# michaelwfc/distributed-tensorflow-resnet

Hardware: AMD Instinct MI355X
Metric: steps/sec (global_batch=128 CIFAR-10 / 1024 ImageNet) ResNet-50 at 1/2/4/8 MI355X (higher is better)
Workload: dtype bf16; 1 GPU; model=resnet50_v2_cifar10, global_batch=128, per_gpu_batch=128, image_size=32, parallelism=dp1, allreduce_dtype=fp32, roctx=False, device=AMD Radeon Graphics, graph=False, wgrad_stream=False, persist_overlap=False, cus=256

## Files before the change

distributed_tensorflow_resnet_amd/csrc/prn_bwd.hip:

```cpp
#include "prn_device.h"

namespace dtr {

namespace {

__device__ __forceinline__ WLoad wl_dgrad(const bf16* src, int co, int ci, int ks) {
  const int K = ks * ks * co;
  return WLoad{src, ci, K, kpad_of(K), 1, ci, co, __frcp_rn((float)(K / 8)), __builtin_ctz(co / 8),
               __builtin_ctz(ci)};
}

template <int SO, int P, int CO, bool PROJ>
__device__ __forceinline__ void dgrad_s2_acc(f32x4 (&acc)[8], const bf16* hal, const bf16* wl,
                                             int kslice, int wave, int lane) {
  using G = Stg<SO, P>;
  lane = opaque_v(lane);
  static_assert(G::CLS, "class-major output");
  if (!wave_active<SO, P>(wave)) return;
  constexpr int RL = G::R / 2, RSL = G::RS / 2, W2L = RL + 2, UL = CO / 8;
  constexpr int KP = kpad_of(PROJ ? CO : 9 * CO);
  const int fr = lane & 15, fq = lane >> 4;
  int pb0, cb0;
  tile_of<SO, P>(wave, 0, pb0, cb0);
  const int cls = (pb0 * 16) / (G::NPX / 4);
// ... 45 lines not shown
                lds16(hal + haddr<G::U>(lr * G::W2 + lc, lc, u * 8)));
  }
}

__device__ __forceinline__ void bn_prefetch_bwd(const PrnBn& bn, int C, BnRegs& r) {
  const int c = threadIdx.x;
  if (c < C) {
    r.g = ldg(bn.gamma + c);
    r.mean = ldg(bn.mean + c);
    r.rstd = ldg(bn.rstd + c);
    r.scale = ldg(bn.scale + c);
    r.shift = ldg(bn.shift + c);
  }
}

__device__ __forceinline__ void bn_prefetch_tab(const PrnBn& bn, int C, BnRegs& r) {
  const int c = threadIdx.x;
  if (c < C) {
    r.scale = ldg(bn.scale + c);
    r.shift = ldg(bn.shift + c);
    r.mean = ldg(bn.mean + c);
    r.rstd = ldg(bn.rstd + c);
  }
}
__device__ __forceinline__ void tab_store(const BnRegs& r, int C, float* tbl) {
  const int c = threadIdx.x;
  if (c < C) {
    tbl[c] = r.scale;
    tbl[64 + c] = r.shift;
    tbl[128 + c] = -r.mean * r.rstd;
    tbl[192 + c] = r.rstd;
  }
}

__device__ __forceinline__ void bn_bwd_table(const PrnBn& bn, const BnRegs& pr, int C, float M,
                                             float* tbl) {
  const int c = threadIdx.x;
  if (c < C) {
    double d1, d2;
    acc_read(bn.bacc, C, c, d1, d2);
    const float sg = (float)d1, sgx = (float)d2;
    const float a = pr.g * pr.rstd;
    const float b = a * sg / M, cc = a * sgx / M;
    tbl[c] = a;
    tbl[64 + c] = cc * pr.mean * pr.rstd - b;
    tbl[128 + c] = -cc * pr.rstd;
    tbl[192 + c] = pr.scale;
    tbl[256 + c] = pr.shift;
    if (blockIdx.x == 0) {
      st_sc1_f32(bn.dbeta + c, sg);
      st_sc1_f32(bn.dgamma + c, sgx);
    }
  }
  __syncthreads();
}

__device__ __forceinline__ void bn_load_table(const PrnBn& bn, int C, float* tbl) {
  const int c = threadIdx.x;
  if (c < C) {
    const float rs = ldg(bn.rstd + c);
    tbl[c] = ldg(bn.scale + c);
    tbl[64 + c] = ldg(bn.shift + c);
    tbl[128 + c] = -ldg(bn.mean + c) * rs;
    tbl[192 + c] = rs;
  }
}

__device__ __forceinline__ float bwd1(float da, float xf, const float* cf, int c) {
  const float gg = fmaf(xf, cf[192 + c], cf[256 + c]) > 0.f ? da : 0.f;
  return fmaf(cf[128 + c], xf, fmaf(cf[c], gg, cf[64 + c]));
}
__device__ __forceinline__ bf16x8 bwd8(bf16x8 da, bf16x8 x, bf16x8 add, bool has_add,
                                       const float* cf, int c0) {
  bf16x8 o;
#pragma unroll
  for (int j = 0; j < 8; ++j) {
    float r = bwd1((float)da[j], (float)x[j], cf, c0 + j);
    if (has_add) r += (float)add[j];
    o[j] = (bf16)r;
  }
  return o;
}

__device__ __forceinline__ void arrive_bwd(Ctx& x) {
  grid_arrive(x.a->bar + PRN_BWD, x.a->shards);
  if (x.mark != nullptr) {
    if (threadIdx.x == 0) __hip_atomic_fetch_add(x.mark, 1u, __ATOMIC_RELAXED, __HIP_MEMORY_SCOPE_AGENT);
    x.mark = nullptr;
  }
}
__device__ __forceinline__ bool wait_bwd(Ctx& x) {
  ++x.nbar;
  const bool ok = grid_wait(x.a->bar, PRN_BWD, x.nbar, x.slices, x.a->shards, x.a->err, x.m.flag);
  if (ok && blockIdx.x == 0 && threadIdx.x == 0)
    __hip_atomic_store(x.a->bar + PRN_READY, x.nbar, __ATOMIC_RELAXED, __HIP_MEMORY_SCOPE_AGENT);
  return ok;
}

template <int S, int P>
__device__ __forceinline__ void bwd_sums(Ctx& x, const bf16x4 (&da)[8], const bf16x4 (&xs)[8],
                                         const float* tb, int bi, int wave, int lane) {
  lane = opaque_v(lane);
  bn_sums<S, P>([&](int t, int r, float& s1, float& s2) {
    int pb, cb;
    tile_of<S, P>(wave, t, pb, cb);
    const int c = cb * 16 + 4 * (lane >> 4) + r;
    const float xf = (float)xs[t][r];
    const float gg = (xf * tb[c] + tb[64 + c] > 0.f) ? (float)da[t][r] : 0.f;
    s1 = gg;
    s2 = gg * fmaf(xf, tb[192 + c], tb[128 + c]);
  }, x.m.red, ld_const(x.a->bns + (bi)).bacc, wave, lane);
}

template <int S, int P, bool ADD>
__device__ __forceinline__ void bwd_apply(bf16x4 (&out)[8], const bf16x4 (&da)[8],
                                          const bf16x4 (&xs)[8], const bf16x4 (&add)[8],
                                          const float* cf, int wave, int lane) {
  lane = opaque_v(lane);
  if (!wave_active<S, P>(wave)) return;
#pragma unroll
  for (int t = 0; t < Stg<S, P>::TPW; ++t) {
    int pb, cb;
    tile_of<S, P>(wave, t, pb, cb);
#pragma unroll
    for (int r = 0; r < 4; ++r) {
      const int c = cb * 16 + 4 * (lane >> 4) + r;
      float o = bwd1((float)da[t][r], (float)xs[t][r], cf, c);
      if (ADD) o += (float)add[t][r];
      out[t][r] = (bf16)o;
    }
  }
}

struct NbrBwd {
  bf16x8 dv, xv, av;
};
template <int S, int P>
__device__ __forceinline__ void bwd_nbr_issue(const Nbr<S, P>& nb, const bf16* da,
                                              const bf16* xsrc, const bf16* add, NbrBwd& q) {
  if ((int)threadIdx.x < Nbr<S, P>::UNITS && nb.ok) {
    q.dv = da ? ld_sc1_b128(da, nb.gofs) : bf16x8{};
    q.xv = ldg(reinterpret_cast<const bf16x8*>(xsrc + nb.gofs));
    q.av = add ? ld_sc1_b128(add, nb.gofs) : bf16x8{};
  }
}
template <int S, int P>
__device__ __forceinline__ void bwd_halo(Ctx& x, bf16* hal, const bf16x4 (&own)[8],
                                         const Nbr<S, P>& nb, NbrBwd& q, const float* dpc,
                                         bool has_add, const float* cf, int wave, int lane) {
  bf16x8 nv = {};
  if ((int)threadIdx.x < Nbr<S, P>::UNITS && nb.ok) {
    if (dpc) {
#pragma unroll
      for (int j = 0; j < 8; ++j) q.dv[j] = (bf16)dpc[nb.u * 8 + j];
    }
    nv = bwd8(q.dv, q.xv, q.av, has_add, cf, nb.u * 8);
  }
  to_halo<S, P, 0>(hal, own, nullptr, nullptr, nb, nv, x.kslice, wave, lane);
}

template <int S, int STR, bool PROJ, int P>
__device__ __forceinline__ bool block_bwd(Ctx& x, bf16x4 (&dout)[8], bf16x4 (&hs)[8],
                                          const WLoad& next_w2, bool has_prev,
                                          const PrnBlock& Bn, const PrnBlock& B) {
  constexpr int SI = STR == 2 ? S - 1 : S;
  using GI = Stg<SI, P>;
  using G = Stg<S, P>;
  const PrnArgs& a = *x.a;
  const int wave = opaque_s(x.wave), lane = opaque_v(x.lane);
  const long img_o = (long)x.img * G::R * G::R * G::C;
  const long img_i = (long)x.img * GI::R * GI::R * GI::C;
  probe(x, 100 + S);
  bf16x4 xs[8];
  load_regs<SI, P>(xs, B.x + img_i, x.kslice, wave, lane);
  tab_store(x.ftr, G::C, x.m.tbl);
  __syncthreads();
  probe(x, 1);
  f32x4 acc[8];
  zero_acc(acc);
  conv_acc<S, P, G::C, 3, 1, true>(acc, x.m.hb, x.m.w1, x.kslice, wave, lane, x.m.red);
  bf16x4 da[8];
  round_acc<S, P, false>(da, acc, da);
  probe(x, 3);
  if constexpr (P > 1)
    publish<S, P, 1>(da, B.da2 + img_o, x.kslice, wave, lane);
  bwd_sums<S, P>(x, da, hs, x.m.tbl, B.bn2, wave, lane);
  probe(x, 4);
  arrive_bwd(x);
  {
    const WLoad L1 = wl_dgrad(B.w1b, G::C, GI::C, 3);
    WLoad LP{};
    if (PROJ) LP = wl_dgrad(B.wpb, G::C, GI::C, 1);
    bf16x8 w1r[nreg(conv_units(G::C, GI::C, 3))], wpr[1];
    w_prefetch(L1, w1r);
    w_prefetch(LP, wpr);
    bn_prefetch_bwd(ld_const(a.bns + (B.bn2)), G::C, x.bnr);
    bn_prefetch_tab(ld_const(a.bns + (B.bn1)), GI::C, x.ftr);
    halo_to_global<S, P>(x.m.hb, B.dout + img_o, x.kslice);
    probe(x, 5);
    if (!wait_bwd(x)) return false;
    probe(x, 6);
    const Nbr<S, P> nb(x.kslice);
    NbrBwd q;
    bwd_nbr_issue<S, P>(nb, B.da2 + img_o, B.h1 + img_o, nullptr, q);
    bn_bwd_table(ld_const(a.bns + (B.bn2)), x.bnr, G::C, (float)a.N * G::R * G::R, x.m.tbl2);
    bf16x4 dh[8];
    bwd_apply<S, P, false>(dh, da, hs, dh, x.m.tbl2, wave, lane);
    bwd_halo<S, P>(x, x.m.ha, dh, nb, q, nullptr, false, x.m.tbl2, wave, lane);
    tab_store(x.ftr, GI::C, x.m.tbl);
    w_store(L1, w1r, x.m.w1);
    w_store(LP, wpr, x.m.w2);
  }
  __syncthreads();
  probe(x, 8);
  zero_acc(acc);
  if constexpr (STR == 2) {
    dgrad_s2_acc<SI, P, G::C, false>(acc, x.m.ha, x.m.w1, x.kslice, wave, lane);
    dgrad_s2_acc<SI, P, G::C, true>(acc, x.m.hb, x.m.w2, x.kslice, wave, lane);
  } else {
    conv_acc<S, P, G::C, 3, 1, true>(acc, x.m.ha, x.m.w1, x.kslice, wave, lane, x.m.red);
    if constexpr (PROJ) conv_acc<S, P, G::C, 1, 1, false>(acc, x.m.hb, x.m.w2, x.kslice, wave, lane, x.m.red);
  }
  round_acc<SI, P, false>(da, acc, da);
  probe(x, 9);
  if constexpr (P > 1)
    publish<SI, P, 1>(da, B.da1 + img_i, x.kslice, wave, lane);
  bwd_sums<SI, P>(x, da, xs, x.m.tbl, B.bn1, wave, lane);
  probe(x, 10);
  arrive_bwd(x);
  halo_to_global<S, P>(x.m.ha, B.dh1 + img_o, x.kslice);
  probe(x, 11);
  bf16x8 w2r[nreg(conv_units(G::C, G::C, 3))];
  w_prefetch(next_w2, w2r);
  bn_prefetch_bwd(ld_const(a.bns + (B.bn1)), GI::C, x.bnr);
  if (has_prev) bn_prefetch_tab(ld_const(a.bns + (Bn.bn2)), GI::C, x.ftr);
  if (!wait_bwd(x)) return false;
  probe(x, 12);
  const Nbr<SI, P> nb(x.kslice);
  NbrBwd q;
  bwd_nbr_issue<SI, P>(nb, B.da1 + img_i, B.x + img_i, PROJ ? nullptr : B.dout + img_o, q);
  bn_bwd_table(ld_const(a.bns + (B.bn1)), x.bnr, GI::C, (float)a.N * GI::R * GI::R, x.m.tbl2);
  probe(x, 13);
  if (PROJ && a.overlap && blockIdx.x == 0 && a.bucket_of_stage[S] >= 0)
    x.mark = a.bar + PRN_BUCKET + a.bucket_of_stage[S] * PRN_LINE;
  if constexpr (PROJ) bwd_apply<SI, P, false>(dout, da, xs, dout, x.m.tbl2, wave, lane);
  else bwd_apply<SI, P, true>(dout, da, xs, dout, x.m.tbl2, wave, lane);
  probe(x, 14);
  if (has_prev) load_regs<SI, P>(hs, Bn.h1 + img_i, x.kslice, wave, lane);
  bwd_halo<SI, P>(x, x.m.hb, dout, nb, q, nullptr, !PROJ, x.m.tbl2, wave, lane);
  probe(x, 15);
  w_store(next_w2, w2r, x.m.w1);
  return true;
}

template <int CO, int CI, int KSZ, int STR, int RO, int WT>
__device__ __forceinline__ void wgrad_item(const PrnItem& it, char* smem, int wave, int lane, bool wt) {
  constexpr int RI = RO * STR, W2 = RI + 2, OFF = KSZ == 1 ? 1 : 0;
  constexpr int KN = KSZ * KSZ * CI, NB = (KN + 15) / 16, MB = CO / 16;
  constexpr int TILES = MB * NB, TPW = TILES / WT, WKS = NW / WT;
  constexpr int KSI = RO * RO / 32, KPW = KSI / WKS;
  static_assert(TILES % WT == 0 && KSI % WKS == 0 && TPW <= 36, "wgrad tiles");
  static_assert(NB % TPW == 0, "a wave's tiles share one output-channel block");
  bf16* dys = reinterpret_cast<bf16*>(smem);
  bf16* hal = dys + RO * RO * CO;
  float* tb = reinterpret_cast<float*>(hal + W2 * W2 * CI);
  const int tid = threadIdx.x;
  wave = opaque_s(wave);
  lane = opaque_v(lane);
  const int tg = wave % WT, kq = wave / WT;
  const int gq = lane >> 4, li = lane & 15, qr = li >> 2, pc = li & 3;
  if (it.scale != nullptr && tid < CI) {
    tb[tid] = ldg(it.scale + tid);
    tb[64 + tid] = ldg(it.shift + tid);
  }
  f32x4 acc[TPW];
#pragma unroll
  for (int t = 0; t < TPW; ++t) acc[t] = f32x4{0.f, 0.f, 0.f, 0.f};
  constexpr int DU = RO * RO * CO / 8, CU = CI / 8, XU = W2 * W2 * CU;
  constexpr int ND = (DU + PT - 1) / PT, NX = (XU + PT - 1) / PT;
  bf16x8 rd[ND], rx[NX];
  auto fetch = [&](int n) {
#pragma unroll
    for (int i = 0; i < ND; ++i) {
      const int q = tid + i * PT;
      if (q < DU) rd[i] = ld_sc1_b128(it.dy, (long)n * RO * RO * CO + q * 8);
    }
#pragma unroll
    for (int i = 0; i < NX; ++i) {
      const int q = tid + i * PT, pix = q / CU, u = q - pix * CU;
      const int hr = pix / W2, hc = pix - hr * W2;
      rx[i] = bf16x8{};
      if (q < XU && hr >= 1 && hr <= RI && hc >= 1 && hc <= RI)
        rx[i] = ldg(reinterpret_cast<const bf16x8*>(it.x + (((long)n * RI + hr - 1) * RI + hc - 1) * CI + u * 8));
    }
  };
  const int nend = it.img0 + it.nimg;
  fetch(it.img0);
  for (int n = it.img0; n < nend; ++n) {
    __syncthreads();
#pragma unroll
    for (int i = 0; i < ND; ++i) {
      const int q = tid + i * PT;
      if (q < DU) *reinterpret_cast<bf16x8*>(dys + q * 8) = rd[i];
    }
#pragma unroll
    for (int i = 0; i < NX; ++i) {
      const int q = tid + i * PT, pix = q / CU, u = q - pix * CU;
      const int hr = pix / W2, hc = pix - hr * W2;
      if (q < XU) {
        bf16x8 v = rx[i];
        if (it.scale != nullptr && hr >= 1 && hr <= RI && hc >= 1 && hc <= RI)
          v = affine_relu8(v, tb + u * 8, tb + 64 + u * 8);
// ... 57 lines not shown
    for (int t = 0; t < TPW; ++t) {
      const int tile = tg * TPW + t, mb = tile / NB, nb = tile - mb * NB;
      const int n = nb * 16 + li;
      if (n < KN) {
        if (wt) {
#pragma unroll
          for (int i = 0; i < 4; ++i) st_sc1_f32(it.part + (long)(mb * 16 + 4 * gq + i) * KN + n, acc[t][i]);
        } else {
#pragma unroll
          for (int i = 0; i < 4; ++i) stg(it.part + (long)(mb * 16 + 4 * gq + i) * KN + n, acc[t][i]);
        }
      }
    }
  }
  __syncthreads();
}

constexpr int PRN_KINDS = 9;
__host__ __device__ constexpr int wg_lds(int co, int ci, int str, int ro) {
  return ro * ro * co * 2 + (ro * str + 2) * (ro * str + 2) * ci * 2 + 512;
}

__device__ __forceinline__ void run_item(const PrnItem& it, char* smem, int wave, int lane, bool wt) {
  switch (it.kind) {
    case 0: wgrad_item<16, 16, 3, 1, 32, 1>(it, smem, wave, lane, wt); break;
    case 1: wgrad_item<32, 32, 3, 1, 16, 2>(it, smem, wave, lane, wt); break;
    case 2: wgrad_item<64, 64, 3, 1, 8, 8>(it, smem, wave, lane, wt); break;
    case 3: wgrad_item<32, 16, 3, 2, 16, 2>(it, smem, wave, lane, wt); break;
    case 4: wgrad_item<64, 32, 3, 2, 8, 8>(it, smem, wave, lane, wt); break;
    case 5: wgrad_item<16, 16, 1, 1, 32, 1>(it, smem, wave, lane, wt); break;
    case 6: wgrad_item<32, 16, 1, 2, 16, 2>(it, smem, wave, lane, wt); break;
    case 7: wgrad_item<64, 32, 1, 2, 8, 8>(it, smem, wave, lane, wt); break;
    case 8: wgrad_item<16, 8, 3, 1, 32, 1>(it, smem, wave, lane, wt); break;
    default: break;
  }
}


}

template <int P>
__device__ __forceinline__ bool prn_bwd_slices(const PrnArgs& a, char* smem, int wave, int lane) {
  const int nsl = a.N * P;
  const int tid = threadIdx.x;
  Ctx x;
  x.a = &a;
  x.m = carve(smem);
  x.img = blockIdx.x / P;
  x.kslice = blockIdx.x % P;
  x.wave = wave;
  x.lane = lane;
  x.nbar = 0;
  x.slices = (unsigned)nsl;
  x.pc = 0;
  x.mark = nullptr;
  probe(x, 0);
  const int nb = a.nblocks;
  const PrnBlock& BL = ld_const(a.blocks + (nb - 1));
  {
    const WLoad L = wl_dgrad(BL.w2b, 64, 64, 3);
    bf16x8 r[nreg(conv_units(64, 64, 3))];
    w_prefetch(L, r);
    w_store(L, r, x.m.w1);
  }
  using G2 = Stg<2, P>;
  bf16x4 dout[8], hs[8];
  {
    const int fb = 2 * nb;
    const long img_o = (long)x.img * 64 * 64;
    bf16x4 xs[8];
    load_regs<2, P>(xs, BL.out + img_o, x.kslice, wave, lane);
    float* dps = x.m.tbl + 256;
    bn_load_table(ld_const(a.bns + (fb)), 64, x.m.tbl);
    if (tid < 64) dps[tid] = a.dpool[(long)x.img * 64 + tid];
    __syncthreads();
    bf16x4 dp[8];
#pragma unroll
    for (int t = 0; t < G2::TPW; ++t) {
      int pb, cb;
      tile_of<2, P>(wave, t, pb, cb);
#pragma unroll
      for (int r = 0; r < 4; ++r) dp[t][r] = (bf16)dps[(cb * 16 + 4 * (lane >> 4) + r) & 63];
    }
    bwd_sums<2, P>(x, dp, xs, x.m.tbl, fb, wave, lane);
    arrive_bwd(x);
    bn_prefetch_bwd(ld_const(a.bns + (fb)), 64, x.bnr);
    bn_prefetch_tab(ld_const(a.bns + (BL.bn2)), 64, x.ftr);
    if (!wait_bwd(x)) return false;
    const Nbr<2, P> nb(x.kslice);
    NbrBwd q;
    bwd_nbr_issue<2, P>(nb, nullptr, BL.out + img_o, nullptr, q);
    bn_bwd_table(ld_const(a.bns + (fb)), x.bnr, 64, (float)a.N * 64, x.m.tbl2);
    bwd_apply<2, P, false>(dout, dp, xs, dout, x.m.tbl2, wave, lane);
    load_regs<2, P>(hs, BL.h1 + img_o, x.kslice, wave, lane);
    bwd_halo<2, P>(x, x.m.hb, dout, nb, q, dps, false, x.m.tbl2, wave, lane);
  }
  const int nps = nb / 3;
  auto run = [&](auto tag, int bi) -> bool {
    constexpr int S = decltype(tag)::S, STR = decltype(tag)::STR;
    constexpr bool PROJ = decltype(tag)::PROJ;
    WLoad n2{};
    const bool hp = bi > 0;
    const PrnBlock Bp = ld_const(a.blocks + (hp ? bi - 1 : bi));
    if (hp) n2 = wl_dgrad(Bp.w2b, 16 << Bp.stage, 16 << Bp.stage, 3);
    return block_bwd<S, STR, PROJ, P>(x, dout, hs, n2, hp, Bp, ld_const(a.blocks + (bi)));
  };
  for (int bi = nb - 1; bi > 2 * nps; --bi)
    if (!run(BlkTag<2, 1, false>{}, bi)) return false;
  if (!run(BlkTag<2, 2, true>{}, 2 * nps)) return false;
  for (int bi = 2 * nps - 1; bi > nps; --bi)
    if (!run(BlkTag<1, 1, false>{}, bi)) return false;
  if (!run(BlkTag<1, 2, true>{}, nps)) return false;
  for (int bi = nps - 1; bi > 0; --bi)
    if (!run(BlkTag<0, 1, false>{}, bi)) return false;
  if (!run(BlkTag<0, 1, true>{}, 0)) return false;
  probe(x, 200);
  if constexpr (P == 1) {
    __syncthreads();
    halo_to_global<0, P>(x.m.hb, a.dx0 + (long)x.img * 1024 * 16, x.kslice);
  } else {
    publish<0, P>(dout, a.dx0 + (long)x.img * 1024 * 16, x.kslice, wave, lane);
  }
  arrive_bwd(x);
  if (blockIdx.x == 0) wait_bwd(x);
  return true;
}

__device__ void prn_head_fold(const PrnArgs& a, char* smem, int tid) {
  const int N = a.N, ld = a.kpad, classes = a.classes;
  float* red = reinterpret_cast<float*>(smem);
  float* sw = red + 256;
  bf16* sp = reinterpret_cast<bf16*>(sw + ((N * ld + 3 * N + 3) & ~3));
  bf16* sd = sp + N * 64;
  for (int i = tid; i < N * ld / 4; i += PT)
    reinterpret_cast<f32x4*>(sw)[i] = ldg(reinterpret_cast<const f32x4*>(a.ws) + i);
  for (int i = tid; i < N; i += PT)
    reinterpret_cast<float2*>(sw + N * ld)[i] = ldg(reinterpret_cast<const float2*>(a.ws + N * ld) + i);
  if (a.topk_out != nullptr)
    for (int i = tid; i < N; i += PT) sw[N * ld + 2 * N + i] = ldg(a.ws + N * ld + 2 * N + i);
  for (int i = tid; i < N * 8; i += PT)
    reinterpret_cast<uint4*>(sp)[i] = ldg(reinterpret_cast<const uint4*>(a.pooled) + i);
  for (int i = tid; i < N * ld / 8; i += PT)
    reinterpret_cast<uint4*>(sd)[i] = ldg(reinterpret_cast<const uint4*>(a.dlogits) + i);
  __syncthreads();
  const int lane = tid & 63, q = tid >> 6;
  if (q < 4) {
    float t = 0.f;
    if (lane < classes) {
#pragma unroll 8
      for (int r = q; r < N; r += 4) t += sw[r * ld + lane];
    }
    red[q * 64 + lane] = t;
  } else if (q == 4) {
    const float* rs = sw + N * ld;
    float l = 0.f, k = 0.f;
    for (int r = lane; r < N; r += 64) {
      l += rs[2 * r];
      k += rs[2 * r + 1];
    }
    l = wave_sum(l);
    k = wave_sum(k);
    if (lane == 0) {
      stg(a.loss_sum, l);
      stg(a.correct, k);
    }
    if (a.topk_out != nullptr) {
      const float* rk = rs + 2 * N;
      float k5 = 0.f;
// ... 164 lines not shown
```

distributed_tensorflow_resnet_amd/csrc/prn_device.h:

```cpp
#pragma once
#include <algorithm>
#include <stdexcept>

#include "common.h"
#include "kernels.h"

namespace dtr {

namespace {

constexpr int PT = PRN_THREADS;
constexpr int NW = PT / 64;
constexpr long long kSpinTicks = 200000000;

typedef unsigned u32x2 __attribute__((ext_vector_type(2)));
typedef unsigned u32x4 __attribute__((ext_vector_type(4)));

template <int S, int P>
struct Stg {
  static constexpr int R = 32 >> S, C = 16 << S, U = C / 8, W2 = R + 2;
  static constexpr int RS = R / P, HR = RS + 2;
  static constexpr int NPX = R * RS;
  static constexpr int NPB = NPX / 16, NCB = C / 16;
  static constexpr int WPB = NPB >= NW ? 1 : NW / NPB;
// ... 361 lines not shown
    const bool border = lr == 0 || lr == G::RS - 1;
    if (ROWS == 0 || (ROWS == 1) == border) {
      if constexpr (WB) st_wb_b64(img_base, (h * G::R + w) * G::C + cb * 16 + 4 * (lane >> 4), v[t]);
      else st_sc1_b64(img_base, (h * G::R + w) * G::C + cb * 16 + 4 * (lane >> 4), v[t]);
    }
  }
}

template <int S, int P>
struct Nbr {
  static constexpr int UNITS = 2 * Stg<S, P>::R * Stg<S, P>::U;
  static_assert(UNITS <= PT, "neighbour units");
  int sel, col, u, gofs;
  bool ok;
  __device__ __forceinline__ Nbr(int kslice) {
    using G = Stg<S, P>;
    const int t = threadIdx.x;
    sel = t / (G::R * G::U);
    const int rem = t - sel * G::R * G::U;
    col = rem / G::U;
    u = rem - col * G::U;
    const int gr = sel ? (kslice + 1) * G::RS : kslice * G::RS - 1;
    ok = t < UNITS && gr >= 0 && gr < G::R;
    gofs = (gr * G::R + col) * G::C + u * 8;
  }
};

template <int S, int P, int MODE>
__device__ __forceinline__ void to_halo(bf16* hal, const bf16x4 (&v)[8], const float* sc,
                                        const float* sh, const Nbr<S, P>& nb, bf16x8 nv,
                                        int kslice, int wave, int lane) {
  using G = Stg<S, P>;
  lane = opaque_v(lane);
  const int fr = lane & 15, fq = lane >> 4;
  if (wave_active<S, P>(wave)) {
    f32x4 scv[G::CBW], shv[G::CBW];
    if constexpr (MODE == 1) {
#pragma unroll
      for (int j = 0; j < G::CBW; ++j) {
        int pb, cb;
        tile_of<S, P>(wave, j, pb, cb);
        scv[j] = *reinterpret_cast<const f32x4*>(sc + cb * 16 + 4 * fq);
        shv[j] = *reinterpret_cast<const f32x4*>(sh + cb * 16 + 4 * fq);
      }
    }
#pragma unroll
    for (int t = 0; t < G::TPW; ++t) {
      int pb, cb, h, w;
      tile_of<S, P>(wave, t, pb, cb);
      canon<S, P>(kslice, pb * 16 + fr, h, w);
      const int c0 = cb * 16 + 4 * fq;
      bf16x4 o = v[t];
      if constexpr (MODE == 1) {
#pragma unroll
        for (int r = 0; r < 4; ++r)
          o[r] = (bf16)fmaxf((float)v[t][r] * scv[t % G::CBW][r] + shv[t % G::CBW][r], 0.f);
      }
      const int lr = h - kslice * G::RS + 1;
      *reinterpret_cast<bf16x4*>(hal + haddr<G::U>(lr * G::W2 + w + 1, w + 1, c0)) = o;
    }
  }
  if ((int)threadIdx.x < Nbr<S, P>::UNITS) {
    const int lr = nb.sel ? G::RS + 1 : 0, lc = nb.col + 1;
    *reinterpret_cast<bf16x8*>(hal + haddr<G::U>(lr * G::W2 + lc, lc, nb.u * 8)) = nb.ok ? nv : bf16x8{};
  }
  for (int q = threadIdx.x; q < 2 * G::HR * G::U; q += PT) {
    const int b = q / G::U, u = q - b * G::U;
    const int lr = b >> 1, lc = (b & 1) ? G::R + 1 : 0;
    *reinterpret_cast<bf16x8*>(hal + haddr<G::U>(lr * G::W2 + lc, lc, u * 8)) = bf16x8{};
  }
}

template <int CTRL>
__device__ __forceinline__ float dpp_mov(float v) {
  return __builtin_bit_cast(float, __builtin_amdgcn_mov_dpp(__builtin_bit_cast(int, v), CTRL, 0xF, 0xF, true));
}
__device__ __forceinline__ float row16_sum(float v) {
  v += dpp_mov<0xB1>(v);
  v += dpp_mov<0x4E>(v);
  v += dpp_mov<0x141>(v);
  v += dpp_mov<0x140>(v);
  return v;
}

constexpr int PRN_ACC_REP = 4;

template <int S, int P, typename F>
__device__ __forceinline__ void bn_sums(F f, float* red, double* acc, int wave, int lane) {
  using G = Stg<S, P>;
  lane = opaque_v(lane);
  const int fr = lane & 15, fq = lane >> 4;
  if (wave_active<S, P>(wave)) {
    float s1[G::CBW][4], s2[G::CBW][4];
#pragma unroll
    for (int j = 0; j < G::CBW; ++j)
#pragma unroll
      for (int r = 0; r < 4; ++r) s1[j][r] = s2[j][r] = 0.f;
#pragma unroll
    for (int t = 0; t < G::TPW; ++t)
#pragma unroll
      for (int r = 0; r < 4; ++r) {
        float a, b;
        f(t, r, a, b);
        s1[t % G::CBW][r] += a;
        s2[t % G::CBW][r] += b;
      }
#pragma unroll
    for (int j = 0; j < G::CBW; ++j)
#pragma unroll
      for (int r = 0; r < 4; ++r) {
        s1[j][r] = row16_sum(s1[j][r]);
        s2[j][r] = row16_sum(s2[j][r]);
      }
    if (fr == 0) {
      int pb, cb0;
      tile_of<S, P>(wave, 0, pb, cb0);
#pragma unroll
      for (int j = 0; j < G::CBW; ++j)
#pragma unroll
        for (int r = 0; r < 4; ++r) {
          const int c = (cb0 + j) * 16 + 4 * fq + r;
          red[wave * 128 + c] = s1[j][r];
          red[wave * 128 + 64 + c] = s2[j][r];
        }
    }
  }
  __syncthreads();
  if (threadIdx.x < G::C) {
    const int c = threadIdx.x;
    const int grp = (c / 16) / G::CBW;
    float v1 = 0.f, v2 = 0.f;
#pragma unroll
    for (int w = 0; w < NW; ++w)
      if (w % G::WPB == grp) {
        v1 += red[w * 128 + c];
        v2 += red[w * 128 + 64 + c];
      }
    double* p = acc + (long)(blockIdx.x % PRN_ACC_REP) * 2 * G::C + c;
    atomic_add_g(p, (double)v1);
    atomic_add_g(p + G::C, (double)v2);
  }
}

__device__ __forceinline__ void acc_read(const double* acc, int C, int c, double& s1, double& s2) {
  double a[PRN_ACC_REP], b[PRN_ACC_REP];
#pragma unroll
  for (int r = 0; r < PRN_ACC_REP; ++r) {
    a[r] = ld_sc1_d(acc + (long)r * 2 * C + c);
    b[r] = ld_sc1_d(acc + (long)r * 2 * C + C + c);
  }
  s1 = s2 = 0.0;
#pragma unroll
  for (int r = 0; r < PRN_ACC_REP; ++r) {
    s1 += a[r];
    s2 += b[r];
  }
}

struct BnRegs {
  float g, b, mean, rstd, scale, shift, mm, mv;
};
__device__ __forceinline__ void bn_prefetch_fwd(const PrnBn& bn, int C, BnRegs& r) {
  const int c = threadIdx.x;
  if (c < C) {
    r.g = ldg(bn.gamma + c);
    r.b = ldg(bn.beta + c);
    if (blockIdx.x == 0) {
      r.mm = ldg(bn.mmean + c);
      r.mv = ldg(bn.mvar + c);
    }
  }
}

__device__ __forceinline__ void bn_fwd_table(const PrnBn& bn, const BnRegs& pr, int C, double M,
                                             float eps, float momentum, int update_moving,
                                             float* tbl) {
  const int c = threadIdx.x;
  if (c < C) {
    double s1, s2;
    acc_read(bn.acc, C, c, s1, s2);
    const double dm = s1 / M;
    const double var = fmax(s2 / M - dm * dm, 0.0);
    const float fmu = (float)dm, fvar = (float)var;
    const float rs = rsqrtf(fvar + eps);
    const float sc = pr.g * rs;
    const float sh = pr.b - fmu * sc;
    tbl[c] = sc;
    tbl[64 + c] = sh;
    tbl[128 + c] = fmu;
    tbl[192 + c] = rs;
    if (blockIdx.x == 0) {
      stg(bn.mean + c, fmu);
      stg(bn.rstd + c, rs);
      stg(bn.scale + c, sc);
      stg(bn.shift + c, sh);
      if (update_moving) {
        const float uvar = M > 1.0 ? (float)(var * M / (M - 1.0)) : fvar;
        const float mm = pr.mm, mv = pr.mv;
        stg(bn.mmean + c, mm - (1.f - momentum) * (mm - fmu));
        stg(bn.mvar + c, mv - (1.f - momentum) * (mv - uvar));
      }
    }
  }
  __syncthreads();
}

constexpr int HALO_B = (32 + 2) * 34 * 16 * 2;
constexpr int W1_B = 64 * kpad_of(576) * 2;
constexpr int W2_B = 64 * kpad_of(32) * 2;
constexpr int TBL_B = 7 * 64 * 4;
constexpr int RED_B = 8 * 128 * 4;
constexpr int MISC_B = 256;
constexpr int OFF_HA = 0, OFF_HB = OFF_HA + HALO_B, OFF_W1 = OFF_HB + HALO_B,
              OFF_W2 = OFF_W1 + W1_B, OFF_TBL = OFF_W2 + W2_B, OFF_TBL2 = OFF_TBL + TBL_B,
              OFF_RED = OFF_TBL2 + TBL_B, OFF_MISC = OFF_RED + RED_B,
              LDS_TOTAL = OFF_MISC + MISC_B;
static_assert(LDS_TOTAL <= 163840, "LDS");

struct Smem {
  bf16 *ha, *hb, *w1, *w2;
  float *tbl, *tbl2, *red;
  int* flag;
};
// ... 144 lines not shown
```

distributed_tensorflow_resnet_amd/csrc/prn_fwd.hip:

```cpp
#include "prn_device.h"
#include "xent_row.h"

namespace dtr {

namespace {

__device__ __forceinline__ bool wait_fwd(Ctx& x) {
  ++x.nbar;
  if (x.a->fault_bar == (int)x.nbar && blockIdx.x == 0) {
    if (threadIdx.x == 0) __hip_atomic_store(x.a->err, 2, __ATOMIC_RELAXED, __HIP_MEMORY_SCOPE_AGENT);
    return false;
  }
  return grid_wait(x.a->bar, PRN_FWD, x.nbar, x.slices, x.a->shards, x.a->err, x.m.flag);
}

template <int S, int P>
__device__ __forceinline__ void fwd_sums(Ctx& x, const bf16x4 (&v)[8], int bi, int wave, int lane) {
  bn_sums<S, P>([&](int t, int r, float& s1, float& s2) {
    const float f = (float)v[t][r];
    s1 = f;
    s2 = f * f;
  }, x.m.red, ld_const(x.a->bns + (bi)).acc, wave, lane);
}

template <int S, int P>
__device__ __forceinline__ void fwd_bn_halo(Ctx& x, bf16* hal, const bf16x4 (&v)[8],
                                            const bf16* src, int bi, int wave, int lane) {
  using G = Stg<S, P>;
  const PrnArgs& a = *x.a;
  const Nbr<S, P> nb(x.kslice);
  bf16x8 nv = {};
  if ((int)threadIdx.x < Nbr<S, P>::UNITS && nb.ok) nv = ld_sc1_b128(src, nb.gofs);
  bn_fwd_table(ld_const(a.bns + (bi)), x.bnr, G::C, (double)a.N * G::R * G::R, a.eps, a.momentum,
               a.update_moving, x.m.tbl);
  if ((int)threadIdx.x < Nbr<S, P>::UNITS && nb.ok)
    nv = affine_relu8(nv, x.m.tbl + nb.u * 8, x.m.tbl + 64 + nb.u * 8);
  to_halo<S, P, 1>(hal, v, x.m.tbl, x.m.tbl + 64, nb, nv, x.kslice, wave, lane);
}

template <int S, int STR, bool PROJ, int P>
__device__ __forceinline__ bool block_fwd(Ctx& x, bf16x4 (&xr)[8], int bi_next,
                                          const WLoad& next_w1, const WLoad& next_wp,
                                          const PrnBlock& B) {
  constexpr int SI = STR == 2 ? S - 1 : S;
  using GI = Stg<SI, P>;
  using G = Stg<S, P>;
  const PrnArgs& a = *x.a;
  const int wave = opaque_s(x.wave), lane = opaque_v(x.lane);
  const long img_o = (long)x.img * G::R * G::R * G::C;
  const long img_i = (long)x.img * GI::R * GI::R * GI::C;
  probe(x, 100 + S);
  fwd_bn_halo<SI, P>(x, x.m.ha, xr, B.x + img_i, B.bn1, wave, lane);
  probe(x, 1);
  __syncthreads();
  probe(x, 2);
  bf16x4 pr[8], hr[8];
  f32x4 acc[8];
  if constexpr (PROJ) {
    zero_acc(acc);
    conv_acc<S, P, GI::C, 1, STR, false>(acc, x.m.ha, x.m.w2, x.kslice, wave, lane, x.m.red);
    round_acc<S, P, false>(pr, acc, pr);
  }
  zero_acc(acc);
  conv_acc<S, P, GI::C, 3, STR, false>(acc, x.m.ha, x.m.w1, x.kslice, wave, lane, x.m.red);
  round_acc<S, P, false>(hr, acc, hr);
  probe(x, 3);
  if constexpr (P > 1) publish<S, P, 1>(hr, B.h1 + img_o, x.kslice, wave, lane);
  fwd_sums<S, P>(x, hr, B.bn2, wave, lane);
  probe(x, 4);
  grid_arrive(a.bar + PRN_FWD, a.shards);
  publish<S, P, P == 1 ? 0 : 2, true>(hr, B.h1 + img_o, x.kslice, wave, lane);
  probe(x, 5);
  {
    bf16x8 w2r[nreg(conv_units(G::C, G::C, 3))];
    const WLoad L2 = wl_fwd(B.w2f, G::C, G::C, 3);
    w_prefetch(L2, w2r);
    bn_prefetch_fwd(ld_const(a.bns + (B.bn2)), G::C, x.bnr);
    if (!wait_fwd(x)) return false;
    probe(x, 6);
    fwd_bn_halo<S, P>(x, x.m.ha, hr, B.h1 + img_o, B.bn2, wave, lane);
    w_store(L2, w2r, x.m.w1);
  }
  __syncthreads();
  probe(x, 8);
  zero_acc(acc);
  conv_acc<S, P, G::C, 3, 1, false>(acc, x.m.ha, x.m.w1, x.kslice, wave, lane, x.m.red);
  if constexpr (PROJ) round_acc<S, P, true>(xr, acc, pr);
  else round_acc<S, P, true>(xr, acc, xr);
  probe(x, 9);
  if constexpr (P > 1) publish<S, P, 1>(xr, B.out + img_o, x.kslice, wave, lane);
  fwd_sums<S, P>(x, xr, bi_next, wave, lane);
  probe(x, 10);
  grid_arrive(a.bar + PRN_FWD, a.shards);
  publish<S, P, P == 1 ? 0 : 2, true>(xr, B.out + img_o, x.kslice, wave, lane);
  probe(x, 11);
  bf16x8 w1r[nreg_next_fwd<S>()], wpr[1];
  w_prefetch(next_w1, w1r);
  w_prefetch(next_wp, wpr);
  bn_prefetch_fwd(ld_const(a.bns + (bi_next)), G::C, x.bnr);
  if (!wait_fwd(x)) return false;
  probe(x, 12);
  w_store(next_w1, w1r, x.m.w1);
  w_store(next_wp, wpr, x.m.w2);
  return true;
}

template <int P>
__device__ __forceinline__ void prn_forward_body(const PrnArgs& a, char* smem) {
  Ctx x;
  x.a = &a;
  x.m = carve(smem);
  x.img = blockIdx.x / P;
  x.kslice = blockIdx.x % P;
  x.wave = __builtin_amdgcn_readfirstlane(threadIdx.x >> 6);
  x.lane = threadIdx.x & 63;
  x.nbar = 0;
  x.slices = (unsigned)(a.N * P);
  x.pc = 0;
  x.mark = nullptr;
  const int tid = threadIdx.x;
  probe(x, 0);

  stem_fill<P, false>(a, x.img, x.m.ha, x.m.w1, x.kslice);
  __syncthreads();
  const PrnBlock& B0 = ld_const(a.blocks + (0));
  bf16x4 xr[8];
  {
    f32x4 acc[8];
    zero_acc(acc);
    conv_acc<0, P, 8, 3, 1, false>(acc, x.m.ha, x.m.w1, x.kslice, x.wave, x.lane, x.m.red);
    round_acc<0, P, false>(xr, acc, xr);
    if constexpr (P > 1) publish<0, P, 1>(xr, B0.x + (long)x.img * 1024 * 16, x.kslice, x.wave, x.lane);
    fwd_sums<0, P>(x, xr, B0.bn1, x.wave, x.lane);
    grid_arrive(a.bar + PRN_FWD, a.shards);
    publish<0, P, P == 1 ? 0 : 2, true>(xr, B0.x + (long)x.img * 1024 * 16, x.kslice, x.wave, x.lane);
    const WLoad L1 = wl_fwd(B0.w1f, 16, 16, 3);
    WLoad LP{};
    if (B0.wpf) LP = wl_fwd(B0.wpf, 16, 16, 1);
    bf16x8 w1r[nreg(conv_units(16, 16, 3))], wpr[1];
    w_prefetch(L1, w1r);
    w_prefetch(LP, wpr);
    bn_prefetch_fwd(ld_const(a.bns + (B0.bn1)), 16, x.bnr);
    if (!wait_fwd(x)) return;
    w_store(L1, w1r, x.m.w1);
    w_store(LP, wpr, x.m.w2);
  }

  const int nps = a.nblocks / 3;
  auto run = [&](auto tag, int bi) -> bool {
    constexpr int S = decltype(tag)::S, STR = decltype(tag)::STR;
    constexpr bool PROJ = decltype(tag)::PROJ;
    const PrnBlock& B = ld_const(a.blocks + (bi));
    const bool last = bi + 1 == a.nblocks;
    const int bnx = last ? 2 * a.nblocks : ld_const(a.blocks + (bi + 1)).bn1;
    WLoad n1{}, np{};
    if (!last) {
      const PrnBlock& Bn = ld_const(a.blocks + (bi + 1));
      const int so = Bn.stage, si = Bn.stride == 2 ? so - 1 : so;
      n1 = wl_fwd(Bn.w1f, 16 << so, 16 << si, 3);
      if (Bn.wpf) np = wl_fwd(Bn.wpf, 16 << so, 16 << si, 1);
    }
    return block_fwd<S, STR, PROJ, P>(x, xr, bnx, n1, np, B);
  };
  if (!run(BlkTag<0, 1, true>{}, 0)) return;
  for (int bi = 1; bi < nps; ++bi)
    if (!run(BlkTag<0, 1, false>{}, bi)) return;
  if (!run(BlkTag<1, 2, true>{}, nps)) return;
  for (int bi = nps + 1; bi < 2 * nps; ++bi)
    if (!run(BlkTag<1, 1, false>{}, bi)) return;
  if (!run(BlkTag<2, 2, true>{}, 2 * nps)) return;
  for (int bi = 2 * nps + 1; bi < 3 * nps; ++bi)
    if (!run(BlkTag<2, 1, false>{}, bi)) return;

  probe(x, 200);
  const int fb = 2 * a.nblocks;
  const int dunits = 64 * a.kpad / 8;
  bf16x8 dwv = {};
  if (x.kslice == 0 && tid < dunits) dwv = *reinterpret_cast<const bf16x8*>(a.dense_w + tid * 8);
  bn_fwd_table(ld_const(a.bns + (fb)), x.bnr, 64, (double)a.N * 64, a.eps, a.momentum, a.update_moving, x.m.tbl);
  {
    const float v = pool_sums<P>(xr, x.m.tbl, x.m.red, x.wave, x.lane);
    if (tid < 64) atomic_add_g(a.pool_acc + (long)x.img * 64 + tid, (double)v);
  }
  grid_arrive(a.bar + PRN_FWD, a.shards);
  if (!wait_fwd(x)) return;
  if (x.kslice != 0) return;
  float* pool_s = x.m.tbl2;
  float* wd = reinterpret_cast<float*>(x.m.w1);
  if (tid < dunits)
#pragma unroll
    for (int j = 0; j < 8; ++j) wd[tid * 8 + j] = (float)dwv[j];
  if (tid < 64) {
    const bf16 pb = (bf16)((float)ld_sc1_d(a.pool_acc + (long)x.img * 64 + tid) / 64.f);
    a.pooled[(long)x.img * 64 + tid] = pb;
    pool_s[tid] = (float)pb;
  }
  __syncthreads();
  if (x.wave == 0) {
    const int lane = x.lane;
    const int y = a.labels[x.img];
    float z = -INFINITY;
    if (lane < a.classes) {
      float acc = 0.f;
#pragma unroll 8
      for (int c = 0; c < 64; ++c) acc += pool_s[c] * wd[c * a.kpad + lane];
      z = acc + a.dense_b[lane];
    }
    const float zy = __shfl(z, (y >= 0 && y < a.classes) ? y : 0, 64);
    const XentRow r = xent_row<1>([&](int) { return z; }, lane, a.classes, y, zy,
                                  a.label_smoothing, a.topk);
    float g = 0.f;
    if (lane < a.classes) g = r.grad(r.prob(z), lane == y, a.grad_scale);
    if (lane < a.kpad) {
      const bf16 gb = (bf16)g;
      a.dlogits[(long)x.img * a.kpad + lane] = gb;
      a.ws[(long)x.img * a.kpad + lane] = g;
      pool_s[128 + lane] = (float)gb;
// ... 66 lines not shown
```

Baseline: 1348 steps/s.

## Fuse BN statistic reduction with grid barrier arrive and batch DPP reductions

The BN sum reduction now interleaves its DPP row reductions across all accumulators and writes partial sums with vector stores. The cross-wave reduce is split across more threads. With P==1, the arrive is done by wave 0 right after its own atomics drain, instead of a full grid_arrive after a block-wide sync. The goal is to shorten the critical path between the end of the BN statistic atomics and the barrier signal in every forward and backward stage. The risk is memory-ordering subtleties, since the arrive relies on vmcnt waits rather than a full block barrier.

```diff
diff --git a/distributed_tensorflow_resnet_amd/csrc/prn_bwd.hip b/distributed_tensorflow_resnet_amd/csrc/prn_bwd.hip
--- a/distributed_tensorflow_resnet_amd/csrc/prn_bwd.hip
+++ b/distributed_tensorflow_resnet_amd/csrc/prn_bwd.hip
@@ -151,12 +151,15 @@
   return o;
 }
 
-__device__ __forceinline__ void arrive_bwd(Ctx& x) {
-  grid_arrive(x.a->bar + PRN_BWD, x.a->shards);
+__device__ __forceinline__ void mark_bwd(Ctx& x) {
   if (x.mark != nullptr) {
     if (threadIdx.x == 0) __hip_atomic_fetch_add(x.mark, 1u, __ATOMIC_RELAXED, __HIP_MEMORY_SCOPE_AGENT);
     x.mark = nullptr;
   }
+}
+__device__ __forceinline__ void arrive_bwd(Ctx& x) {
+  grid_arrive(x.a->bar + PRN_BWD, x.a->shards);
+  mark_bwd(x);
 }
 __device__ __forceinline__ bool wait_bwd(Ctx& x) {
   ++x.nbar;
@@ -167,8 +170,8 @@
 }
 
 template <int S, int P>
-__device__ __forceinline__ void bwd_sums(Ctx& x, const bf16x4 (&da)[8], const bf16x4 (&xs)[8],
-                                         const float* tb, int bi, int wave, int lane) {
+__device__ __forceinline__ void bwd_sums_arrive(Ctx& x, const bf16x4 (&da)[8], const bf16x4 (&xs)[8],
+                                                const float* tb, int bi, int tag, int wave, int lane) {
   lane = opaque_v(lane);
   bn_sums<S, P>([&](int t, int r, float& s1, float& s2) {
     int pb, cb;
@@ -179,6 +182,9 @@
     s1 = gg;
     s2 = gg * fmaf(xf, tb[192 + c], tb[128 + c]);
   }, x.m.red, ld_const(x.a->bns + (bi)).bacc, wave, lane);
+  if (tag) probe(x, tag);
+  bn_sums_arrive<P>(x.a->bar + PRN_BWD, x.a->shards, wave);
+  mark_bwd(x);
 }
 
 template <int S, int P, bool ADD>
@@ -253,9 +259,8 @@
   probe(x, 3);
   if constexpr (P > 1)
     publish<S, P, 1>(da, B.da2 + img_o, x.kslice, wave, lane);
-  bwd_sums<S, P>(x, da, hs, x.m.tbl, B.bn2, wave, lane);
-  probe(x, 4);
-  arrive_bwd(x);
+  if constexpr (P > 1) probe(x, 20);
+  bwd_sums_arrive<S, P>(x, da, hs, x.m.tbl, B.bn2, 4, wave, lane);
   {
     const WLoad L1 = wl_dgrad(B.w1b, G::C, GI::C, 3);
     WLoad LP{};
@@ -294,9 +299,8 @@
   probe(x, 9);
   if constexpr (P > 1)
     publish<SI, P, 1>(da, B.da1 + img_i, x.kslice, wave, lane);
-  bwd_sums<SI, P>(x, da, xs, x.m.tbl, B.bn1, wave, lane);
-  probe(x, 10);
-  arrive_bwd(x);
+  if constexpr (P > 1) probe(x, 21);
+  bwd_sums_arrive<SI, P>(x, da, xs, x.m.tbl, B.bn1, 10, wave, lane);
   halo_to_global<S, P>(x.m.ha, B.dh1 + img_o, x.kslice);
   probe(x, 11);
   bf16x8 w2r[nreg(conv_units(G::C, G::C, 3))];
@@ -520,8 +524,7 @@
 #pragma unroll
       for (int r = 0; r < 4; ++r) dp[t][r] = (bf16)dps[(cb * 16 + 4 * (lane >> 4) + r) & 63];
     }
-    bwd_sums<2, P>(x, dp, xs, x.m.tbl, fb, wave, lane);
-    arrive_bwd(x);
+    bwd_sums_arrive<2, P>(x, dp, xs, x.m.tbl, fb, 0, wave, lane);
     bn_prefetch_bwd(ld_const(a.bns + (fb)), 64, x.bnr);
     bn_prefetch_tab(ld_const(a.bns + (BL.bn2)), 64, x.ftr);
     if (!wait_bwd(x)) return false;
diff --git a/distributed_tensorflow_resnet_amd/csrc/prn_device.h b/distributed_tensorflow_resnet_amd/csrc/prn_device.h
--- a/distributed_tensorflow_resnet_amd/csrc/prn_device.h
+++ b/distributed_tensorflow_resnet_amd/csrc/prn_device.h
@@ -467,63 +467,88 @@
   v += dpp_mov<0x140>(v);
   return v;
 }
+template <int N>
+__device__ __forceinline__ void row16_sum_n(float (&v)[N]) {
+#pragma unroll
+  for (int i = 0; i < N; ++i) v[i] += dpp_mov<0xB1>(v[i]);
+#pragma unroll
+  for (int i = 0; i < N; ++i) v[i] += dpp_mov<0x4E>(v[i]);
+#pragma unroll
+  for (int i = 0; i < N; ++i) v[i] += dpp_mov<0x141>(v[i]);
+#pragma unroll
+  for (int i = 0; i < N; ++i) v[i] += dpp_mov<0x140>(v[i]);
+}
 
 constexpr int PRN_ACC_REP = 4;
 
 template <int S, int P, typename F>
 __device__ __forceinline__ void bn_sums(F f, float* red, double* acc, int wave, int lane) {
   using G = Stg<S, P>;
+  constexpr int C = G::C;
+  constexpr int SPT = 2 * C > 64 ? 2 : 1, NTH = 2 * C / SPT;
+  constexpr int NCH = NW / G::WPB;
+  constexpr bool SELF = P == 1;
   lane = opaque_v(lane);
   const int fr = lane & 15, fq = lane >> 4;
   if (wave_active<S, P>(wave)) {
-    float s1[G::CBW][4], s2[G::CBW][4];
-#pragma unroll
-    for (int j = 0; j < G::CBW; ++j)
-#pragma unroll
-      for (int r = 0; r < 4; ++r) s1[j][r] = s2[j][r] = 0.f;
+    float s[2 * G::CBW * 4];
+#pragma unroll
+    for (int i = 0; i < 2 * G::CBW * 4; ++i) s[i] = 0.f;
 #pragma unroll
     for (int t = 0; t < G::TPW; ++t)
 #pragma unroll
       for (int r = 0; r < 4; ++r) {
         float a, b;
         f(t, r, a, b);
-        s1[t % G::CBW][r] += a;
-        s2[t % G::CBW][r] += b;
-      }
-#pragma unroll
-    for (int j = 0; j < G::CBW; ++j)
-#pragma unroll
-      for (int r = 0; r < 4; ++r) {
-        s1[j][r] = row16_sum(s1[j][r]);
-        s2[j][r] = row16_sum(s2[j][r]);
-      }
+        s[(t % G::CBW) * 4 + r] += a;
+        s[(G::CBW + t % G::CBW) * 4 + r] += b;
+      }
+    row16_sum_n(s);
     if (fr == 0) {
       int pb, cb0;
       tile_of<S, P>(wave, 0, pb, cb0);
 #pragma unroll
-      for (int j = 0; j < G::CBW; ++j)
-#pragma unroll
-        for (int r = 0; r < 4; ++r) {
-          const int c = (cb0 + j) * 16 + 4 * fq + r;
-          red[wave * 128 + c] = s1[j][r];
-          red[wave * 128 + 64 + c] = s2[j][r];
-        }
-    }
-  }
+      for (int j = 0; j < G::CBW; ++j) {
+        float* q = red + wave * 128 + (cb0 + j) * 16 + 4 * fq;
+        *reinterpret_cast<f32x4*>(q) = f32x4{s[j * 4], s[j * 4 + 1], s[j * 4 + 2], s[j * 4 + 3]};
+        *reinterpret_cast<f32x4*>(q + C) = f32x4{s[(G::CBW + j) * 4], s[(G::CBW + j) * 4 + 1],
+                                                 s[(G::CBW + j) * 4 + 2], s[(G::CBW + j) * 4 + 3]};
+      }
+    }
+  }
+  if constexpr (SELF) asm volatile("s_waitcnt vmcnt(0)" ::: "memory");
   __syncthreads();
-  if (threadIdx.x < G::C) {
-    const int c = threadIdx.x;
-    const int grp = (c / 16) / G::CBW;
-    float v1 = 0.f, v2 = 0.f;
-#pragma unroll
-    for (int w = 0; w < NW; ++w)
-      if (w % G::WPB == grp) {
-        v1 += red[w * 128 + c];
-        v2 += red[w * 128 + 64 + c];
-      }
-    double* p = acc + (long)(blockIdx.x % PRN_ACC_REP) * 2 * G::C + c;
-    atomic_add_g(p, (double)v1);
-    atomic_add_g(p + G::C, (double)v2);
+  if (threadIdx.x < NTH) {
+    float ld[SPT][NCH];
+#pragma unroll
+    for (int k = 0; k < SPT; ++k) {
+      const int i = threadIdx.x + k * NTH;
+      const int grp = ((i & (C - 1)) / 16) / G::CBW;
+#pragma unroll
+      for (int q = 0; q < NCH; ++q) ld[k][q] = red[(grp + q * G::WPB) * 128 + i];
+    }
+    double* p = acc + (long)(blockIdx.x % PRN_ACC_REP) * 2 * C + threadIdx.x;
+#pragma unroll
+    for (int k = 0; k < SPT; ++k) {
+      float v = 0.f;
+#pragma unroll
+      for (int q = 0; q < NCH; ++q) v += ld[k][q];
+      atomic_add_g(p + k * NTH, (double)v);
+    }
+  }
+}
+
+template <int P>
+__device__ __forceinline__ void bn_sums_arrive(unsigned* bar, int shards, int wave) {
+  if constexpr (P == 1) {
+    if (wave == 0) {
+      asm volatile("s_waitcnt vmcnt(0)" ::: "memory");
+      if (threadIdx.x == 0)
+        __hip_atomic_fetch_add(bar + (blockIdx.x % shards) * PRN_LINE, 1u, __ATOMIC_RELAXED,
+                               __HIP_MEMORY_SCOPE_AGENT);
+    }
+  } else {
+    grid_arrive(bar, shards);
   }
 }
 
diff --git a/distributed_tensorflow_resnet_amd/csrc/prn_fwd.hip b/distributed_tensorflow_resnet_amd/csrc/prn_fwd.hip
--- a/distributed_tensorflow_resnet_amd/csrc/prn_fwd.hip
+++ b/distributed_tensorflow_resnet_amd/csrc/prn_fwd.hip
@@ -15,12 +15,15 @@
 }
 
 template <int S, int P>
-__device__ __forceinline__ void fwd_sums(Ctx& x, const bf16x4 (&v)[8], int bi, int wave, int lane) {
+__device__ __forceinline__ void fwd_sums_arrive(Ctx& x, const bf16x4 (&v)[8], int bi, int tag,
+                                                int wave, int lane) {
   bn_sums<S, P>([&](int t, int r, float& s1, float& s2) {
     const float f = (float)v[t][r];
     s1 = f;
     s2 = f * f;
   }, x.m.red, ld_const(x.a->bns + (bi)).acc, wave, lane);
+  if (tag) probe(x, tag);
+  bn_sums_arrive<P>(x.a->bar + PRN_FWD, x.a->shards, wave);
 }
 
 template <int S, int P>
@@ -66,9 +69,8 @@
   round_acc<S, P, false>(hr, acc, hr);
   probe(x, 3);
   if constexpr (P > 1) publish<S, P, 1>(hr, B.h1 + img_o, x.kslice, wave, lane);
-  fwd_sums<S, P>(x, hr, B.bn2, wave, lane);
-  probe(x, 4);
-  grid_arrive(a.bar + PRN_FWD, a.shards);
+  if constexpr (P > 1) probe(x, 20);
+  fwd_sums_arrive<S, P>(x, hr, B.bn2, 4, wave, lane);
   publish<S, P, P == 1 ? 0 : 2, true>(hr, B.h1 + img_o, x.kslice, wave, lane);
   probe(x, 5);
   {
@@ -89,9 +91,8 @@
   else round_acc<S, P, true>(xr, acc, xr);
   probe(x, 9);
   if constexpr (P > 1) publish<S, P, 1>(xr, B.out + img_o, x.kslice, wave, lane);
-  fwd_sums<S, P>(x, xr, bi_next, wave, lane);
-  probe(x, 10);
-  grid_arrive(a.bar + PRN_FWD, a.shards);
+  if constexpr (P > 1) probe(x, 21);
+  fwd_sums_arrive<S, P>(x, xr, bi_next, 10, wave, lane);
   publish<S, P, P == 1 ? 0 : 2, true>(xr, B.out + img_o, x.kslice, wave, lane);
   probe(x, 11);
   bf16x8 w1r[nreg_next_fwd<S>()], wpr[1];
@@ -131,8 +132,7 @@
     conv_acc<0, P, 8, 3, 1, false>(acc, x.m.ha, x.m.w1, x.kslice, x.wave, x.lane, x.m.red);
     round_acc<0, P, false>(xr, acc, xr);
     if constexpr (P > 1) publish<0, P, 1>(xr, B0.x + (long)x.img * 1024 * 16, x.kslice, x.wave, x.lane);
-    fwd_sums<0, P>(x, xr, B0.bn1, x.wave, x.lane);
-    grid_arrive(a.bar + PRN_FWD, a.shards);
+    fwd_sums_arrive<0, P>(x, xr, B0.bn1, 0, x.wave, x.lane);
     publish<0, P, P == 1 ? 0 : 2, true>(xr, B0.x + (long)x.img * 1024 * 16, x.kslice, x.wave, x.lane);
     const WLoad L1 = wl_fwd(B0.w1f, 16, 16, 3);
     WLoad LP{};
```

Measured after the change: 1393 steps/s, median of 6. +3.3%, better.
